# lasseufpa/intent_radio_sched_multi_slice

Measured on AMD Instinct MI355X. Metric: env-steps/s (batched TTIs) at mult_slice 10-slice/100-UE; 1->8 GPU scaling [device-policy rollout over batch partitions; step-by-step and learner-in-the-loop schedules beside it], higher is better.
Workload: dtype f64

## Files before the change

include/ranenv.h:

```cpp
#ifndef RANENV_H
#define RANENV_H

#include <stdint.h>

#ifdef __cplusplus
extern "C" {
#endif

#define RANENV_ABI_VERSION 10

enum {
    RANENV_OK = 0,
    RANENV_E_INVALID = -1,
    RANENV_E_HIP = -2,
    RANENV_E_STATE = -3,
    RANENV_E_NOMEM = -4
};

enum { RANENV_POLICY_EXTERNAL = 0, RANENV_POLICY_MARR = 1, RANENV_POLICY_MAPF = 2, RANENV_POLICY_NETWORK = 3, RANENV_POLICY_HEAD_NETWORK = 4 };
enum { RANENV_HEAD_DIST_GAUSS_CLIP = 0, RANENV_HEAD_DIST_GAUSS_TANH = 1 };
enum { RANENV_ACT_TANH = 0, RANENV_ACT_RELU = 1 };
enum { RANENV_NET_IN_OBS = 0, RANENV_NET_IN_MASK_OBS = 1 };
enum { RANENV_NET_F32 = 0, RANENV_NET_BF16 = 1 };
enum { RANENV_INTRA_RR = 0, RANENV_INTRA_PF = 1, RANENV_INTRA_MT = 2, RANENV_INTRA_PER_SLICE = 255 };
// ... 78 lines not shown
    int32_t *step_number;
    int32_t *hist_len;
    int8_t  *mask_inter;
    int8_t  *mask_intra;
    double  *policy_scores;
    int32_t *episode_number;
    int32_t *episodes;
} ranenv_views;

const char *ranenv_last_error(ranenv_handle h);
int ranenv_abi_version(void);

int ranenv_create(const ranenv_config *cfg, ranenv_handle *out);
int ranenv_destroy(ranenv_handle h);

int ranenv_load_scenarios(ranenv_handle h, int32_t first, int32_t count,
                          const ranenv_scenario_tables *host_tables, void *stream);

int ranenv_bind_se_pool(ranenv_handle h, const float *dev_pool, int64_t n_tiles, int64_t tile_stride);
int ranenv_bind_se_pool_quad(ranenv_handle h, const float *dev_pool, int64_t n_tiles, int64_t tile_stride);
int ranenv_se_retile_quad(const float *dev_rb_major, float *dev_quad, int64_t n_tiles, int32_t n_ues, int32_t n_rbs, void *stream);
int ranenv_se_retile_member_lines(const float *dev_pool, int32_t quad, int64_t tile_stride, float *dev_lines, int64_t n_tiles, int32_t n_ues,
                                  int32_t n_rbs, void *stream);
int ranenv_member_line_plan(int32_t n_rbs, int32_t max_lines, int32_t *leaf, int32_t *first_rb, int32_t *groups);
int ranenv_member_lines_row_sums_host(const float *row_lines, int32_t n_rbs, int32_t rb_start, int32_t rb_count, double *full, double *part);
int ranenv_member_lines_owner_tail_sums_host(const float *row_lines, int32_t n_rbs, int32_t rb_start, int32_t rb_count, double *full, double *part,
                                             int32_t *walked_lines);
int ranenv_se_retile_member_lines_packed(const float *dev_pool, int32_t quad, int64_t tile_stride, float *dev_lines, int64_t n_tiles, int32_t n_ues,
                                         int32_t n_rbs, void *stream);
int ranenv_member_lines_packed_layout(int32_t n_ues, int32_t n_rbs, int32_t *walked_lines, int64_t *block_offset, int64_t *tile_bytes);
int ranenv_member_lines_packed_sums_host(const float *walk_lines, const float *tail_slot, int32_t n_rbs, int32_t rb_start, int32_t rb_count, double *full,
                                         double *part);
int ranenv_member_serving_order(uint64_t member_mask, uint64_t holder_mask, int32_t lines_per_ue, int32_t dq, int32_t *slots, int32_t *masked_passes);
int ranenv_bind_traffic_pool(ranenv_handle h, const int32_t *dev_pool, int64_t n_rows);

int ranenv_set_episodes(ranenv_handle h, const ranenv_episode *host_episodes, void *stream);

int ranenv_set_policy(ranenv_handle h, int32_t policy, int32_t fixed_intra);

typedef struct {
    int32_t n_hidden;
    int32_t activation;
    int32_t input_layout;
    int32_t precision;
    int32_t dims[6];
    const float *weight[5];
    const float *bias[5];
} ranenv_mlp;
int ranenv_set_policy_network(ranenv_handle h, const ranenv_mlp *inter, const ranenv_mlp *intra, int32_t stochastic, uint64_t seed,
                              void *stream);
int ranenv_get_policy_actions(ranenv_handle h, double **dev_scores, uint8_t **dev_intra);

int ranenv_set_intra_policy_networks(ranenv_handle h, int32_t n, const ranenv_mlp *const *actors, void *stream);
int ranenv_set_intra_value_networks(ranenv_handle h, int32_t n, const ranenv_mlp *const *critics, void *stream);

int ranenv_set_population(ranenv_handle h, int32_t n_members, const int32_t *host_first_env);
int ranenv_get_population(ranenv_handle h, int32_t *n_members, int32_t *host_first_env);
int ranenv_set_population_policy(ranenv_handle h, int32_t n, const ranenv_mlp *const *inter, const ranenv_mlp *const *intra, int32_t stochastic,
                                 uint64_t seed, void *stream);
int ranenv_set_population_value(ranenv_handle h, int32_t n, const ranenv_mlp *const *inter, const ranenv_mlp *const *intra, void *stream);
int ranenv_set_population_member(ranenv_handle h, int32_t member, const ranenv_mlp *inter, const ranenv_mlp *intra, const ranenv_mlp *v_inter,
                                 const ranenv_mlp *v_intra, void *stream);
int ranenv_population_tiles(int32_t n_members, const int32_t *first_env, int32_t e0, int32_t n_envs, int32_t rows_per_env, int32_t *out_member,
                            int32_t *out_row0, int32_t *out_rows, int32_t *n_tiles);

int ranenv_set_population_policy_mixed(ranenv_handle h, int32_t n, const ranenv_mlp *const *inter, const ranenv_mlp *const *intra, int32_t stochastic,
// ... 218 lines not shown
```

intent_radio_sched_multi_slice_amd/_lib.py:

```python
from __future__ import annotations

import ctypes as C
import os

_HERE = os.path.dirname(os.path.abspath(__file__))
LIB_PATH = os.environ.get("RANENV_LIB") or os.path.join(_HERE, "csrc", "libranenv_hip.so")

ABI_VERSION = 10
POLICY_EXTERNAL, POLICY_MARR, POLICY_MAPF, POLICY_NETWORK, POLICY_HEAD_NETWORK = 0, 1, 2, 3, 4
HEAD_DIST_GAUSS_CLIP, HEAD_DIST_GAUSS_TANH = 0, 1
HEAD_SRC_HEAD, HEAD_SRC_INTER = 0, 1
ACT_TANH, ACT_RELU = 0, 1
NET_IN_OBS, NET_IN_MASK_OBS = 0, 1
NET_F32, NET_BF16 = 0, 1
NET_PRECISIONS = {"f32": NET_F32, "bf16": NET_BF16}
NET_MAX_HIDDEN, NET_MAX_WIDTH = 4, 512
INTRA_RR, INTRA_PF, INTRA_MT, INTRA_PER_SLICE = 0, 1, 2, 255
F_CLEAR_HISTORY_ON_RESET, F_NO_RAW_OUTPUT, F_SYNC_CHECK, F_SCALE_PER_ELEMENT = 0x1, 0x2, 0x4, 0x8
SE_STREAM, SE_GATHER = 0, 1
SLICE_METRIC_COLS = 10
LOAD_SLICE_COLS = 6

class RanEnvError(RuntimeError):
    pass
# ... 115 lines not shown
    "ranenv_set_traffic_generator": (C.c_int, [_P, _I32, C.c_uint64, _I32, _P]),
    "ranenv_set_max_steps": (C.c_int, [_P, _P, _P]),
    "ranenv_set_episode_table": (C.c_int, [_P, _P, _I32, _I32, _P]),
    "ranenv_set_autoreset": (C.c_int, [_P, _I32, _I32, _I32, _I32, C.c_uint64, _P, _P]),
    "ranenv_autoreset": (C.c_int, [_P] + [_P] * 7),
    "ranenv_get_poisson_tables": (C.c_int, [_P, _P, _P]),
    "ranenv_set_partitions": (C.c_int, [_P, _I32]),
    "ranenv_rollout": (C.c_int, [_P, _I32] + [_P] * 5),
    "ranenv_enable_metrics": (C.c_int, [_P, _I32, _P]),
    "ranenv_get_metrics": (C.c_int, [_P, C.POINTER(C.c_void_p), C.POINTER(C.c_void_p), C.POINTER(C.c_void_p), C.POINTER(C.c_int32)]),
    "ranenv_step_range": (C.c_int, [_P, _I32, _I32] + [_P] * 9),
    "ranenv_set_se_mode": (C.c_int, [_P, _I32, _P]),
    "ranenv_get_se_sidecars": (C.c_int, [_P, C.POINTER(C.c_void_p), C.POINTER(C.c_void_p), C.POINTER(C.c_int32)]),
    "ranenv_step_part": (C.c_int, [_P, _I32] + [_P] * 9),
    "ranenv_wait_part": (C.c_int, [_P, _I32, _P]),
    "ranenv_get_partition": (C.c_int, [_P, _I32, C.POINTER(C.c_int32), C.POINTER(C.c_int32)]),
    "ranenv_get_part_stream": (C.c_int, [_P, _I32, C.POINTER(C.c_void_p)]),
    "ranenv_autoreset_part": (C.c_int, [_P, _I32] + [_P] * 7),
    "ranenv_set_option": (C.c_int, [_P, C.c_char_p, _I64]),
    "ranenv_get_option": (C.c_int, [_P, C.c_char_p, C.POINTER(C.c_int64)]),
    "ranenv_profile_work": (C.c_int, [_P, C.POINTER(C.c_int64), C.POINTER(C.c_int64)]),
    "ranenv_bind_se_gather_from_power": (C.c_int, [_P, _P, _I64, _F64, _F64, _P]),
    "ranenv_bind_se_pool_quad": (C.c_int, [_P, _P, _I64, _I64]),
    "ranenv_se_retile_quad": (C.c_int, [_P, _P, _I64, _I32, _I32, _P]),
    "ranenv_packed_step_fits": (C.c_int, [C.POINTER(Config), _I64, _I64]),
    "ranenv_se_retile_member_lines": (C.c_int, [_P, _I32, _I64, _P, _I64, _I32, _I32, _P]),
    "ranenv_member_line_plan": (C.c_int, [_I32, _I32, C.POINTER(C.c_int32), C.POINTER(C.c_int32), C.POINTER(C.c_int32)]),
    "ranenv_member_lines_row_sums_host": (C.c_int, [_P, _I32, _I32, _I32, C.POINTER(C.c_double), C.POINTER(C.c_double)]),
    "ranenv_member_lines_owner_tail_sums_host": (C.c_int, [_P, _I32, _I32, _I32, C.POINTER(C.c_double), C.POINTER(C.c_double), C.POINTER(C.c_int32)]),
    "ranenv_se_retile_member_lines_packed": (C.c_int, [_P, _I32, _I64, _P, _I64, _I32, _I32, _P]),
    "ranenv_member_lines_packed_layout": (C.c_int, [_I32, _I32, C.POINTER(C.c_int32), C.POINTER(C.c_int64), C.POINTER(C.c_int64)]),
    "ranenv_member_lines_packed_sums_host": (C.c_int, [_P, _P, _I32, _I32, _I32, C.POINTER(C.c_double), C.POINTER(C.c_double)]),
    "ranenv_member_serving_order": (C.c_int, [C.c_uint64, C.c_uint64, _I32, _I32, C.POINTER(C.c_int32), C.POINTER(C.c_int32)]),
    "ranenv_selftest_ddiv": (C.c_int, [_P, _P, _P, _P, _I64, _P]),
    "ranenv_set_policy_network": (C.c_int, [_P, C.POINTER(Mlp), C.POINTER(Mlp), _I32, C.c_uint64, _P]),
    "ranenv_get_policy_actions": (C.c_int, [_P, C.POINTER(C.c_void_p), C.POINTER(C.c_void_p)]),
    "ranenv_set_value_network": (C.c_int, [_P, C.POINTER(Mlp), C.POINTER(Mlp), _P]),
    "ranenv_collect": (C.c_int, [_P, _I32, C.POINTER(Trajectory), _F64, _F64] + [_P] * 5),
    "ranenv_gae": (C.c_int, [_P, _I32, _I32, _P, _P, _P, _F64, _F64, _P, _P, _P]),
    "ranenv_set_head_policy_network": (C.c_int, [_P, C.POINTER(Mlp), _I32, _P, _I32, C.c_uint64, _P]),
    "ranenv_set_head_value_network": (C.c_int, [_P, C.POINTER(Mlp), _P]),
    "ranenv_get_head_metrics": (C.c_int, [_P, C.POINTER(C.c_void_p), C.POINTER(C.c_void_p), C.POINTER(C.c_int32)]),
    "ranenv_collect_head": (C.c_int, [_P, _I32, C.POINTER(HeadTrajectory), _I32, _F64, _F64] + [_P] * 5),
    "ranenv_enable_slice_metrics": (C.c_int, [_P, _I32, _P]),
    "ranenv_get_slice_metrics": (C.c_int, [_P, C.POINTER(C.c_void_p), C.POINTER(C.c_void_p), C.POINTER(C.c_void_p), C.POINTER(C.c_int32)]),
    "ranenv_bind_replay": (C.c_int, [_P, C.POINTER(Replay)]),
    "ranenv_collect_replay": (C.c_int, [_P, _I32] + [_P] * 5),
    "ranenv_get_replay_count": (C.c_int, [_P, C.POINTER(C.c_int64)]),
    "ranenv_replay_sample": (C.c_int, [_P, _I64, C.c_uint64, C.c_uint64, _I32] + [_P] * 7),
    "ranenv_set_sac_critics": (C.c_int, [_P, C.POINTER(Mlp), C.POINTER(Mlp), _P]),
    "ranenv_sac_targets": (C.c_int, [_P, _I64, _P, _P, _P, _F64, _F64, _I32, C.c_uint64, C.c_uint64] + [_P] * 5),
    "ranenv_set_intra_policy_networks": (C.c_int, [_P, _I32, C.POINTER(C.POINTER(Mlp)), _P]),
    "ranenv_set_intra_value_networks": (C.c_int, [_P, _I32, C.POINTER(C.POINTER(Mlp)), _P]),
    "ranenv_set_head_policy_source": (C.c_int, [_P, _I32]),
    "ranenv_build_se_stats": (C.c_int, [_P, _P]),
    "ranenv_get_se_stats": (C.c_int, [_P, C.POINTER(C.c_void_p), C.POINTER(C.c_int64)]),
    "ranenv_rbs_needed": (C.c_int, [_P, _P, _I32, _I32, _P, _P, _P, _P]),
    "ranenv_bind_trace": (C.c_int, [_P, C.POINTER(Trace), _P]),
    "ranenv_get_trace_counts": (C.c_int, [_P, C.POINTER(C.c_void_p), C.POINTER(C.c_void_p)]),
    "ranenv_reset_trace": (C.c_int, [_P, _P]),
    "ranenv_set_population": (C.c_int, [_P, _I32, C.POINTER(C.c_int32)]),
    "ranenv_get_population": (C.c_int, [_P, C.POINTER(C.c_int32), C.POINTER(C.c_int32)]),
    "ranenv_set_population_policy": (C.c_int, [_P, _I32, C.POINTER(C.POINTER(Mlp)), C.POINTER(C.POINTER(Mlp)), _I32, C.c_uint64, _P]),
    "ranenv_set_population_value": (C.c_int, [_P, _I32, C.POINTER(C.POINTER(Mlp)), C.POINTER(C.POINTER(Mlp)), _P]),
    "ranenv_set_population_member": (C.c_int, [_P, _I32] + [C.POINTER(Mlp)] * 4 + [_P]),
    "ranenv_population_tiles": (C.c_int, [_I32, C.POINTER(C.c_int32), _I32, _I32, _I32] + [C.POINTER(C.c_int32)] * 4),
# ... 66 lines not shown
```

intent_radio_sched_multi_slice_amd/csrc/ranenv_host.cpp:

```cpp
#include <algorithm>
#include <cctype>
#include <cmath>
#include <cstdarg>
#include <cstdio>
#include <cstdlib>
#include <cstring>
#include <new>
#include <string>
#include <array>
#include <vector>

#include "ranenv_internal.h"

using namespace ranenv_dev;

namespace {
thread_local std::string g_last_error;
constexpr int N_STEP_BUILDS = SB_PERSIST_TINY + 1;

}

enum NetRole { NET_INTER, NET_INTRA, NET_INTER_VALUE, NET_INTRA_VALUE, NET_HEAD_CLIP, NET_HEAD_TANH, NET_HEAD_VALUE, NET_SAC_Q };
enum NetForm { FORM_ONE, FORM_SLICE, FORM_MEMBER };

// ... 632 lines not shown
int dev_grow(ranenv_handle h, T **buf, int64_t *cap, int64_t count, const char *what)
{
    if (*buf && *cap >= count) return RANENV_OK;
    dev_drop(h, *buf); *buf = nullptr; *cap = 0;
    void *ptr = nullptr;
    const hipError_t e = hipMalloc(&ptr, (size_t)count * sizeof(T));
    if (e != hipSuccess) return fail(h, RANENV_E_NOMEM, "%s (%.3f GB): %s", what, (double)count * sizeof(T) / 1e9, hipGetErrorString(e));
    h->allocs.push_back(ptr);
    *buf = (T *)ptr; *cap = count;
    return RANENV_OK;
}

template <typename Fill>
int se_sidecars_rebuild(ranenv_handle h, size_t nt, Fill fill)
{
    const int U = h->cfg.n_ues, Rp = (h->cfg.n_rbs + 7) & ~7;
    auto drop = [&](void *ptr) { dev_drop(h, ptr); };
    HIP_TRY(h, hipDeviceSynchronize());
    drop(h->d_se_mean); drop(h->d_se_um); h->d_se_mean = nullptr; h->d_se_um = nullptr;
    void *pm = nullptr, *pu = nullptr;
    hipError_t e = hipMalloc(&pm, nt * (size_t)U * sizeof(double));
    if (e == hipSuccess) e = hipMalloc(&pu, nt * (size_t)U * (size_t)Rp * sizeof(float));
    if (e != hipSuccess) {
        if (pm) (void)hipFree(pm);
        return fail(h, RANENV_E_NOMEM, "SE gather sidecars (%zu tiles: %.2f GB): %s", nt,
                    (double)(nt * (size_t)U * (8 + 4 * (size_t)Rp)) / 1e9, hipGetErrorString(e));
    }
    h->allocs.push_back(pm); h->allocs.push_back(pu);
    h->d_se_mean = (double *)pm; h->d_se_um = (float *)pu; h->se_rp = Rp;
    for (size_t t0 = 0; t0 < nt; t0 += 1u << 20) fill(t0, nt - t0 < (1u << 20) ? nt - t0 : (size_t)(1u << 20));
    return RANENV_OK;
}

struct MemberLine { int leaf, rb0, groups; };
void member_leaves(int lo, int n, std::vector<std::pair<int, int>> &out)
{
    if (n <= 128) { out.push_back({lo, n}); return; }
    int n2 = n / 2; n2 -= n2 % 8;
    member_leaves(lo, n2, out); member_leaves(lo + n2, n - n2, out);
}
std::vector<MemberLine> member_line_plan(int R)
{
    std::vector<std::pair<int, int>> leaves;
    member_leaves(0, R, leaves);
    std::vector<MemberLine> plan;
    for (size_t k = 0; k < leaves.size(); k++) {
        const int G = leaves[k].second >> 3;
        for (int c = 0; 4 * c < G; c++) plan.push_back({(int)k, leaves[k].first + 32 * c, G - 4 * c < 4 ? G - 4 * c : 4});
    }
    if (R & 7) plan.push_back({(int)leaves.size() - 1, R - (R & 7), 0});
    return plan;
}
bool member_line_table(int R, MemberLineTable *tb)
{
    const std::vector<MemberLine> plan = member_line_plan(R);
    if (plan.size() > (size_t)MEMBER_LINES_MAX) return false;
    *tb = MemberLineTable{};
    tb->lines = (int)plan.size(); tb->tail = R & 7;
    for (size_t l = 0; l < plan.size(); l++) { tb->rb0[l] = plan[l].rb0; tb->groups[l] = plan[l].groups; }
    return true;
}
void member_leaf_groups(const float *&line, int lo, int n, unsigned s, unsigned c, double &fr, double &gr)
{
    auto in = [&](int r) { return ((unsigned)r - s) < c ? 1.0 : 0.0; };
    double f[8], g[8];
    for (int j = 0; j < 8; j++) { f[j] = 0.0; g[j] = 0.0; }
// ... 337 lines not shown
            const int m = t->param_metric[i * 3 + k];
            if (bmi[(i * 3 + m) * 2]) return fail(h, RANENV_E_INVALID, "scenario %zu slice %zu declares metric %d twice: one parameter per metric and slice", i / S, i % S, m);
            bmi[(i * 3 + m) * 2] = 1; bmi[(i * 3 + m) * 2 + 1] = t->param_op[i * 3 + k]; bmf[i * 3 + m] = t->param_value[i * 3 + k];
        }
        for (int k = 0; k < nues; k++) {
            const int ue = t->slice_ues[i * Us + k];
            if (ue < 0 || ue >= U) return fail(h, RANENV_E_INVALID, "slice_ues entry %d outside [0,%d)", ue, U);
        }
    }
    for (size_t i = 0; i < n; i++) {
        std::vector<char> seen(S, 0);
        for (int s = 0; s < S; s++) seen[t->sorted_slices[i * S + s]] = 1;
        for (int s = 0; s < S; s++) if (!seen[s]) return fail(h, RANENV_E_INVALID, "sorted_slices row %zu is not a permutation", i);
    }
    for (size_t i = 0; i < n * U; i++) {
        if (t->ue_pkt_size[i] <= 0 || t->ue_max_pkts[i] <= 0) return fail(h, RANENV_E_INVALID, "ue_pkt_size / ue_max_pkts must be positive");
        if (t->ue_max_age[i] < 0 || t->ue_max_age[i] > h->cfg.max_age_cap) return fail(h, RANENV_E_INVALID, "ue_max_age %d outside [0, max_age_cap=%d]", t->ue_max_age[i], h->cfg.max_age_cap);
        if (t->ue_slice[i] < -1 || t->ue_slice[i] >= S) return fail(h, RANENV_E_INVALID, "ue_slice %d outside [-1,%d)", t->ue_slice[i], S);
        if (t->ue_pos[i] < 0 || t->ue_pos[i] >= Us) return fail(h, RANENV_E_INVALID, "ue_pos %d outside [0,%d)", t->ue_pos[i], Us);
    }
    const size_t NSL = (size_t)S * GRP;
    std::vector<int32_t> sue(n * NSL, -1), smp(n * NSL, 1), spk(n * NSL, 1);
    for (size_t i = 0; i < n; i++)
        for (int sl = 0; sl < S; sl++)
            for (int k = 0; k < t->slice_nues[i * S + sl]; k++) {
                const int ue = t->slice_ues[(i * S + sl) * Us + k];
                const size_t o = i * NSL + (size_t)sl * GRP + k;
                if (t->ue_slice[i * U + ue] != sl || t->ue_pos[i * U + ue] != k)
                    return fail(h, RANENV_E_INVALID, "scenario %zu: ue_slice/ue_pos disagree with slice_ues", i);
                sue[o] = ue; smp[o] = t->ue_max_pkts[i * U + ue]; spk[o] = t->ue_pkt_size[i * U + ue];
            }
    std::vector<int32_t> lt[N_TUE];
    for (auto &v : lt) v.resize(n * (size_t)U);
    for (size_t i = 0; i < n; i++) {
        int l = 0;
        for (int pass = 0; pass < 2; pass++)
            for (int ue = 0; ue < U; ue++) {
                const size_t o = i * U + ue;
                if ((t->ue_slice[o] >= 0) != (pass == 0)) continue;
                const size_t d = i * U + (size_t)l++;
                lt[0][d] = t->ue_slice[o]; lt[1][d] = t->ue_pos[o]; lt[2][d] = t->ue_pkt_size[o];
                lt[3][d] = t->ue_max_pkts[o]; lt[4][d] = t->ue_max_age[o]; lt[5][d] = ue;
            }
    }
    h->idle_check_dirty = true;
    if (h->members_host.size() != (size_t)h->cfg.n_scenarios) h->members_host.assign((size_t)h->cfg.n_scenarios, 0);
    for (size_t i = 0; i < n; i++) {
        int m = 0;
        for (int ue = 0; ue < U; ue++) m += t->ue_slice[i * U + ue] >= 0 ? 1 : 0;
        h->members_host[(size_t)first + i] = m;
    }
    h->pclass_dirty = true;
    const size_t f = (size_t)first;
    const Tables &d = h->kp.tab;
    const KP &k = h->kp;
#define PUT(dst, src, elems, type) HIP_TRY(h, hipMemcpyAsync((dst), (src), (elems) * sizeof(type), hipMemcpyHostToDevice, stream))
    PUT(d.slice_i32 + f * S * 8, si.data(), n * S * 8, int32_t);
    PUT(d.slice_f64 + f * S * 2, sf.data(), n * S * 2, double);
    PUT(d.param_i32 + f * S * 6, pi.data(), n * S * 6, int32_t);
    PUT(d.param_f64 + f * S * 3, pf.data(), n * S * 3, double);
    PUT(d.param_i32 + ((size_t)h->cfg.n_scenarios + f) * S * 6, bmi.data(), n * S * 6, int32_t);
    PUT(d.param_f64 + ((size_t)h->cfg.n_scenarios + f) * S * 3, bmf.data(), n * S * 3, double);
    PUT(d.slice_ues + f * S * Us, t->slice_ues, n * S * Us, int32_t);
    PUT(TB_ue_slice(k) + f * U, lt[0].data(), n * U, int32_t);
    PUT(TB_ue_pos(k) + f * U, lt[1].data(), n * U, int32_t);
    PUT(TB_ue_pkt_size(k) + f * U, lt[2].data(), n * U, int32_t);
    PUT(TB_ue_max_pkts(k) + f * U, lt[3].data(), n * U, int32_t);
    PUT(TB_ue_max_age(k) + f * U, lt[4].data(), n * U, int32_t);
    PUT(TB_lane_ue(k) + f * U, lt[5].data(), n * U, int32_t);
    {
        const size_t set1 = (size_t)6 * (size_t)k.NSU;
        std::vector<int32_t> ident(n * (size_t)U);
        for (size_t i = 0; i < ident.size(); i++) ident[i] = (int32_t)(i % (size_t)U);
        PUT(TB_ue_slice(k) + set1 + f * U, t->ue_slice, n * U, int32_t);
        PUT(TB_ue_pos(k) + set1 + f * U, t->ue_pos, n * U, int32_t);
        PUT(TB_ue_pkt_size(k) + set1 + f * U, t->ue_pkt_size, n * U, int32_t);
// ... 88 lines not shown
int ranenv_member_line_plan(int32_t n_rbs, int32_t max_lines, int32_t *leaf, int32_t *first_rb, int32_t *groups)
{
    if (n_rbs < 1 || max_lines < 0) return fail(nullptr, RANENV_E_INVALID, "bad sizes");
    const std::vector<MemberLine> plan = member_line_plan((int)n_rbs);
    for (size_t l = 0; l < plan.size() && l < (size_t)max_lines; l++) {
        if (leaf) leaf[l] = plan[l].leaf;
        if (first_rb) first_rb[l] = plan[l].rb0;
        if (groups) groups[l] = plan[l].groups;
    }
    return (int)plan.size();
}

int ranenv_member_serving_order(uint64_t member_mask, uint64_t holder_mask, int32_t lines_per_ue, int32_t dq, int32_t *slots, int32_t *masked_passes)
{
    if (!slots || !masked_passes) return fail(nullptr, RANENV_E_INVALID, "null argument");
    if (lines_per_ue < 1 || dq < 1 || (holder_mask & ~member_mask) != 0) return fail(nullptr, RANENV_E_INVALID, "bad sizes, or a holder that is no member");
    const int p0 = (dq + lines_per_ue - 1) / lines_per_ue;
    if (p0 > 8) return fail(nullptr, RANENV_E_INVALID, "dq %d at %d lines per UE: the prefix exceeds the wave", (int)dq, (int)lines_per_ue);
    const int pre = p0 * 8;
    int top = 0;
    for (int l = 0; l < 64; l++) if (member_mask >> l & 1) top = l + 1;
    int next = pre;
    for (int l = 0; l < pre; l++) slots[l] = l;
    for (int group = 0; group < 3; group++)
        for (int l = pre; l < 64; l++) {
            const bool m = member_mask >> l & 1, hd = holder_mask >> l & 1;
            if ((group == 0 && hd) || (group == 1 && m && !hd) || (group == 2 && !m)) slots[l] = next++;
        }
    int holders_behind = 0;
    for (int l = pre; l < 64; l++) holders_behind += (int)(holder_mask >> l & 1);
    const int passes = (top + 7) / 8, want = p0 + (holders_behind + 7) / 8;
    *masked_passes = want < passes ? want : passes;
    return RANENV_OK;
}

int ranenv_member_lines_row_sums_host(const float *row_lines, int32_t n_rbs, int32_t rb_start, int32_t rb_count, double *full, double *part)
{
    if (!row_lines || !full || !part) return fail(nullptr, RANENV_E_INVALID, "null argument");
    if (n_rbs < 1 || rb_start < 0 || rb_count < 0) return fail(nullptr, RANENV_E_INVALID, "bad sizes");
    const float *line = row_lines;
    member_lines_pairwise(line, 0, (int)n_rbs, (unsigned)rb_start, (unsigned)rb_count, *full, *part);
    return RANENV_OK;
}

static int member_owner_tail_sums(const float *walk, const float *tail8, int R, unsigned s, unsigned c, double *full, double *part)
{
    const int tail = R & 7;
    const float *line = walk;
    std::vector<std::pair<double, double>> left;
    int lo = 0, n = R;
    while (n > 128) {
        int n2 = n / 2; n2 -= n2 % 8;
        double f1, g1;
        member_lines_pairwise(line, lo, n2, s, c, f1, g1);
        left.push_back({f1, g1});
        lo += n2; n -= n2;
    }
    double t, tg;
    member_leaf_groups(line, lo, n, s, c, t, tg);
    const int walked = (int)((line - walk) / 32);
    if (!tail8) tail8 = line;
    for (int k = 0; k < tail; k++) {
        const double d = (double)tail8[k];
        t += d;
        tg = std::fma(d, ((unsigned)(R - tail + k) - s) < c ? 1.0 : 0.0, tg);
    }
// ... 2540 lines not shown
```

intent_radio_sched_multi_slice_amd/csrc/ranenv_internal.h:

```cpp
#pragma once
#include <hip/hip_runtime.h>
#include <hip/hip_ext.h>

#include <cstddef>
#include <cstdint>

#include "ranenv.h"

#ifndef RANENV_DIAG
#define RANENV_DIAG 0
#endif

namespace ranenv_dev {

enum { MODE_STEP = 0, MODE_DENSE = 1, MODE_RESET = 2,
       MODE_PE = 4 };

struct Tables {
    int32_t *slice_i32;
    double  *slice_f64;
    int32_t *param_i32;
    double  *param_f64;
    int32_t *slice_ues;
    int32_t *slot;
    int32_t *slice_usecase;
    int32_t *ue;
};

struct State {
    int32_t *u4;
    int64_t *u8;
    int32_t *b4;
    int2 *age_ring; int32_t *ring_sent; int32_t *ring_drop;
    int8_t *mask_inter, *mask_intra; double *policy_scores;
};
enum { N_U4 = 11, N_U8 = 4, N_B4 = 9, N_TUE = 12 };
#define ST_queue_pkts(p) ((p).st.u4 + (size_t)(0) * (size_t)(p).BU)
#define ST_front(p) ((p).st.u4 + (size_t)(1) * (size_t)(p).BU)
#define ST_front_rem(p) ((p).st.u4 + (size_t)(2) * (size_t)(p).BU)
#define ST_fifo(p) ((p).st.u4 + (size_t)(3) * (size_t)(p).BU)
#define ST_pkt_incoming(p) ((p).st.u4 + (size_t)(4) * (size_t)(p).BU)
#define ST_pkt_throughputs(p) ((p).st.u4 + (size_t)(5) * (size_t)(p).BU)
#define ST_pkt_effective_thr(p) ((p).st.u4 + (size_t)(6) * (size_t)(p).BU)
// ... 322 lines not shown
```

intent_radio_sched_multi_slice_amd/csrc/ranenv_numeric.hpp:

```cpp
#pragma once
#include <type_traits>

#include "ranenv_internal.h"

#define DEVFN __device__ __forceinline__

#ifndef RANENV_FAST_DIV
#define RANENV_FAST_DIV 1
#endif

namespace {
using namespace ranenv_dev;

DEVFN bool d_isclose(double a, double b) { return fabs(a - b) <= (1e-8 + 1e-5 * fabs(b)); }

DEVFN double ddiv(double a, double b)
{
#if RANENV_FAST_DIV
    double r = __builtin_amdgcn_rcp(b);
    double e = fma(-b, r, 1.0);
    r = fma(r, e, r);
    e = fma(-b, r, 1.0);
    r = fma(r, e, r);
    const double q = a * r;
// ... 253 lines not shown
    v4f q[DQ];
    __amdgpu_buffer_rsrc_t rsrc;
    RowPlan pl;
    int blk, nlw, total;
    unsigned my_voff;
    int own_u; bool own_member;
    double fa, ga, fb, gb, ft, gt;
    v4f e0, e1;
    int iq, il;
    unsigned ld_voff;
    DEVFN void issue(v4f &dst)
    {
        if (il == 0)
            ld_voff = (unsigned)__builtin_amdgcn_ds_bpermute((iq * 8 + (int)((threadIdx.x & 63u) >> 3)) * 4, (int)my_voff) + (threadIdx.x & 7u) * 16u;
        dst = __builtin_bit_cast(v4f, __builtin_amdgcn_raw_buffer_load_b128(rsrc, (int)ld_voff, il * 128, SE_AUX_NT));
        if (++il == nlw) { il = 0; iq++; }
    }
    DEVFN void tail_request(int tail)
    {
        const unsigned tv = own_member ? (unsigned)(own_u * 32) : OOB;
        e0 = __builtin_bit_cast(v4f, __builtin_amdgcn_raw_buffer_load_b128(rsrc, (int)tv, blk, SE_AUX_NT));
        if (tail > 4) e1 = __builtin_bit_cast(v4f, __builtin_amdgcn_raw_buffer_load_b128(rsrc, (int)(tv + 16u), blk, SE_AUX_NT));
        else e1 = v4f{0.0f, 0.0f, 0.0f, 0.0f};
    }
    DEVFN void init(const float *tile_lines, int U, int R, bool member, int u)
    {
        pl = make_row_plan(R);
        nlw = member_lines_per_ue(pl, R) - ((R & 7) ? 1 : 0);
        blk = U * nlw * 128;
        rsrc = __builtin_amdgcn_make_buffer_rsrc(const_cast<float *>(tile_lines), 0, blk + ((R & 7) ? U * 32 : 0), 0x00020000);
        const unsigned long long m = __builtin_amdgcn_ballot_w64(member);
        const int top = m != 0 ? 64 - __builtin_clzll(m) : 0;
        total = ((top + 7) >> 3) * nlw;
        my_voff = member ? (unsigned)(u * nlw * 128) : OOB;
        own_u = u; own_member = member;
        iq = 0; il = 0; ld_voff = OOB;
#pragma unroll
        for (int d = 0; d < DQ; d++) if (d < total) issue(q[d]);
    }
};

template <int DQ> DEVFN int member_prefix_passes(int nl) { return (DQ + nl - 1) / nl; }

template <int DQ, typename Hook>
DEVFN void member_line_sums(MemberLines<DQ> &st, int R, unsigned s, unsigned c, Hook after_issue)
{
    typedef typename MemberLines<DQ>::v4f v4f;
    const RowPlan pl = st.pl;
    const int tail = R & 7, nl = st.nlw > 0 ? st.nlw : 1, total = st.total;
    const int j = (int)(threadIdx.x & 7u), cluster = (int)((threadIdx.x & 63u) >> 3);
    const int lane = (int)(threadIdx.x & 63u);
    const bool member = st.own_member;
    const int pre = member_prefix_passes<DQ>(nl) * 8;
    const unsigned long long behind = ~0ull << pre;
    const unsigned long long hb = __builtin_amdgcn_ballot_w64(member && c > 0) & behind;
    const unsigned long long mb = __builtin_amdgcn_ballot_w64(member && c == 0) & behind;
    const unsigned long long nb = behind & ~(hb | mb);
    auto rank = [](unsigned long long m) { return (int)__builtin_amdgcn_mbcnt_hi((unsigned)(m >> 32), __builtin_amdgcn_mbcnt_lo((unsigned)m, 0u)); };
    const int nh = __builtin_popcountll(hb), nm = __builtin_popcountll(mb);
    int slot = lane;
    if (lane >= pre) slot = pre + (!member ? nh + nm + rank(nb) : (c > 0 ? rank(hb) : nh + rank(mb)));
    const int my_sc = (int)(s | (c << 16));
    st.my_voff = (unsigned)__builtin_amdgcn_ds_permute(slot * 4, (int)st.my_voff);
    const int slot_sc = __builtin_amdgcn_ds_permute(slot * 4, my_sc);
    const int my_pass = slot >> 3, my_from = (slot & 7) * 32;
#if RANENV_DIAG == 11
// ... 422 lines not shown
```

intent_radio_sched_multi_slice_amd/csrc/ranenv_step_body.hpp:

```cpp
#pragma once
#include "ranenv_numeric.hpp"

namespace {

#if RANENV_DIAG == 9
#define RANENV_STAMP(k) do { if (!PERSIST && threadIdx.x == 0 && (k) < p.S) \
    ST_policy_scores(p)[(size_t)(p.e0 + blockIdx.x) * p.S + (k)] = (double)__builtin_amdgcn_s_memrealtime(); } while (0)
#elif RANENV_DIAG == 12
#define RANENV_STAMP(k) do { if constexpr (PERSIST) if (tid == 0) { const unsigned long long now_ = __builtin_amdgcn_s_memrealtime(); \
    double *d_ = &ST_policy_scores(p)[(size_t)e * p.S]; \
    if ((k) == 0) { if (warm) acc_add(d_, (double)(now_ - cy.last_stamp)); acc_add(d_ + 9, 1.0); } else acc_add(d_ + (k), (double)(now_ - stamp_prev)); \
    stamp_prev = now_; if ((k) == 8) cy.last_stamp = now_; } } while (0)
#else
#define RANENV_STAMP(k) do { } while (0)
#endif


template <int NP>
struct SharedCore {
    double rows[NP][4 * NP + 2];
    double xr[4][GRP];
    double pf[NP][3];
    double sf[NP][2];
    int si[NP][8];
// ... 446 lines not shown
    RANENV_STAMP(1);

    int do_alloc = 1;
    asm volatile("" : "+s"(do_alloc));
    if (MODE == MODE_STEP && RANENV_DIAG != 7 && do_alloc != 0)
        alloc_front<NP, PACK>(p, sh, tid, e, hlen_old, act && slc >= 0, slc, ue_pos, total, max_pkts, pkt_size, win_sent, sem_prev,
                    rb_start, rb_count, ST_policy_scores(p), narrow);
    RANENV_STAMP(2);

    auto draw_traffic = [&]() -> double {
        if (!(slc >= 0 && sh.si[slc][1] != 0 && sh.sf[slc][1] > 0.0)) return 0.0;
        unsigned rnd[4];
        philox4x32_10((unsigned)(COLD(env_id_base) + e), (unsigned)episode_no, (unsigned)t, (unsigned)u,
                      (unsigned)COLD(trf_seed), (unsigned)(COLD(trf_seed) >> 32), rnd);
        const size_t row = (size_t)sc * S + slc;
        const int k = poisson_draw(COLD(pois_cdf) + row * 256, COLD(pois_guide) + row * 64, ((unsigned long long)rnd[1] << 32) | rnd[0]);
        return (double)k * 1e6;
    };
    if (CARRY && gen_traffic && act) traffic = draw_traffic();

    double my_full = 0.0, my_part = 0.0;
    auto hook = []() {};
    if constexpr (GATHER) {
        if (MODE == MODE_STEP) {
            bool spread = false;
            if constexpr (PACK == 1) {
                unsigned short *desc = reinterpret_cast<unsigned short *>(&sh.xr[0][0]) + (narrow ? 0 : (tid >> 6)) * 64;
                spread = gather_part_spread<PE>(tile, U * p.se_rp * 4, u * p.se_rp * 4, R, (unsigned)rb_start, (unsigned)rb_count, PE ? COLD(bw_per_rb) : 1.0, desc, my_part);
            }
            if (!spread) my_part = gather_part<PACK, GDEPTH, PE>(tile, U * p.se_rp * 4, u * p.se_rp * 4, R, (unsigned)rb_start, (unsigned)rb_count, PE ? COLD(bw_per_rb) : 1.0);
        }
    } else if constexpr (MODE == MODE_STEP) {
        const unsigned us1 = (unsigned)rb_start, uc1 = (unsigned)rb_count;
        if constexpr (MEMBERS) member_line_sums(ml, R, us1, uc1, hook);
        else row_sums<PE>(se1, R, [=](int r) { return ((unsigned)r - us1) < uc1; }, my_full, my_part, hook, PE ? COLD(bw_per_rb) : 1.0);
    } else if constexpr (MODE == MODE_DENSE) {
        const uint8_t *mrow = p.dense + ((size_t)e * U + u) * R;
        row_sums<PE>(se1, R, [=](int r) { return mrow[r] != 0; }, my_full, my_part, hook, PE ? COLD(bw_per_rb) : 1.0);
    } else {
        row_sums(se1, R, [](int) { return false; }, my_full, my_part, hook);
    }
    if constexpr (!STATE_AT_ENTRY) rest_of_state();
    if constexpr (MEMBERS) member_line_finish(ml, R, (unsigned)rb_start, (unsigned)rb_count, my_full, my_part);
    if constexpr (SE_AHEAD && CARRY) {
        if (se_next) {
            const int pos_next = se_pos + 1 >= ep.se_len ? 0 : se_pos + 1;
            asm volatile("" ::: "memory");
            se1.init(p.se_pool + (size_t)(ep.se_base + (long long)pos_next) * (size_t)p.se_stride, U, u, R, se_quad);
            asm volatile("" ::: "memory");
        }
    }
    RANENV_STAMP(3);
    wg_sync(narrow);
    RANENV_STAMP(4);

    double sem_new = 0.0;
    int sent_u = 0, drop_u = 0;
    bool prev_empty = total == 0;
    if (total != 0 && !((double)total > 2e-8 * (double)max_pkts)) prev_empty = d_isclose((double)total / (double)max_pkts, 0.0);
#if RANENV_DIAG == 3
    if (act && my_full < -1.0) {
#else
    if (act) {
#endif
        if (MODE == MODE_DENSE) {
            const uint8_t *mrow = p.dense + ((size_t)e * U + u) * R;
            bool seen = false;
// ... 558 lines not shown
                se_ready = ahead;
                if (k + 1 < n) { warm = true; wg_sync(); }
            }
            done += n;
            full_sync();
            if (tid0 == 0) {
                kp_const_t kc = (kp_const_t)__builtin_amdgcn_kernarg_segment_ptr();
                asm volatile("" : "+s"(kc));
                pl.keep = persist_finish(*kc, pl, e, done, n_tti);
            }
            __syncthreads();
            if (uni(pl.keep) == 0) break;
            warm = true;
        }
    }
}

#ifndef RANENV_CLASS_PRIO
#define RANENV_CLASS_PRIO 1
#endif
#define RANENV_PERSIST_WPE ((NP == 16) ? 4 : 5)
template <bool GATHER, int NP>
__global__ void __launch_bounds__(CORE_NT) __attribute__((amdgpu_waves_per_eu(RANENV_PERSIST_WPE, RANENV_PERSIST_WPE))) ranenv_persist_kernel(const KP p)
{
    (void)p;
#if RANENV_DIAG == 0 || RANENV_DIAG == 12
#if RANENV_CLASS_PRIO
    if ((blockDim.x == WAVE) == GATHER) __builtin_amdgcn_s_setprio(RANENV_CLASS_PRIO);
#endif
    persist_loop<GATHER ? 1 : SE_DEPTH_LEAN, GATHER, NP>();
#endif
}

template <int NP>
__global__ void __launch_bounds__(CORE_NT) __attribute__((amdgpu_waves_per_eu(RANENV_PERSIST_WPE, RANENV_PERSIST_WPE))) ranenv_persist_kernel_members(const KP p)
{
    (void)p;
#if RANENV_DIAG == 0 || RANENV_DIAG == 12
#if RANENV_CLASS_PRIO
    if (blockDim.x != WAVE) __builtin_amdgcn_s_setprio(RANENV_CLASS_PRIO);
#endif
    persist_loop<SE_DEPTH_LEAN, false, NP, true>();
#endif
}

template <int NP>
__global__ void __launch_bounds__(CORE_NT) __attribute__((amdgpu_waves_per_eu(2, 2))) ranenv_persist_kernel_tiny(const KP p)
{
    (void)p;
#if RANENV_DIAG == 0 || RANENV_DIAG == 12
    persist_loop<SE_DEPTH_TINY, false, NP>();
#endif
}

template <int NP>
__global__ void __launch_bounds__(CORE_NT) __attribute__((amdgpu_waves_per_eu(2, 2))) ranenv_core_kernel_tiny1(const KP p)
{
    step_loop<MODE_STEP, SE_DEPTH_TINY, false, NP, false>(p);
}
#define RANENV_CORE_ATTR __attribute__((amdgpu_waves_per_eu(5, 5)))
template <int MODE, int NP, bool MANY>
__global__ void __launch_bounds__(CORE_NT) RANENV_CORE_ATTR ranenv_core_kernel(const KP p)
{
    step_loop<MODE, ((MODE & 3) == MODE_DENSE || NP == 16) ? 1 : SE_DEPTH_LEAN, false, NP, MANY>(p);
}
template <int NP>
__global__ void __launch_bounds__(CORE_NT) __attribute__((amdgpu_waves_per_eu(NP == 16 ? 4 : 5, NP == 16 ? 4 : 5))) ranenv_core_kernel_members(const KP p)
{
    step_loop<MODE_STEP, NP == 16 ? 1 : SE_DEPTH_LEAN, false, NP, true, 1, false, true>(p);
}
template <int MODE, int NP, bool MANY>
__global__ void __launch_bounds__(CORE_NT) __attribute__((amdgpu_waves_per_eu(4, 4))) ranenv_core_kernel_small(const KP p)
{
// ... 21 lines not shown
```

Before: 114.5 million.

## Balance member UEs across waves and prioritise long-walk waves in member line sums

The host-side UE remap no longer packs all slice members into the first lanes. It splits them across waves in 8-lane pass quotas, so each wave walks fewer member-line passes and the per-wave walk lengths are balanced. In the member line-sum phase, waves with longer pass walks raise their hardware priority via s_setprio, then drop back to priority zero after the phase. The members persistent kernel's class-priority condition is made configurable, and an optional pass cap is added but disabled by default. The risks are extra waves doing work, a changed lane layout, and priority churn between waves.

```diff
diff --git a/include/ranenv.h b/include/ranenv.h
--- a/include/ranenv.h
+++ b/include/ranenv.h
@@ -134,6 +134,7 @@
 int ranenv_member_lines_packed_sums_host(const float *walk_lines, const float *tail_slot, int32_t n_rbs, int32_t rb_start, int32_t rb_count, double *full,
                                          double *part);
 int ranenv_member_serving_order(uint64_t member_mask, uint64_t holder_mask, int32_t lines_per_ue, int32_t dq, int32_t *slots, int32_t *masked_passes);
+int ranenv_member_wave_split(int32_t members, int32_t n_ues, int32_t *out_first, int32_t *out_count);
 int ranenv_bind_traffic_pool(ranenv_handle h, const int32_t *dev_pool, int64_t n_rows);
 
 int ranenv_set_episodes(ranenv_handle h, const ranenv_episode *host_episodes, void *stream);
diff --git a/intent_radio_sched_multi_slice_amd/_lib.py b/intent_radio_sched_multi_slice_amd/_lib.py
--- a/intent_radio_sched_multi_slice_amd/_lib.py
+++ b/intent_radio_sched_multi_slice_amd/_lib.py
@@ -171,6 +171,7 @@
     "ranenv_member_lines_packed_layout": (C.c_int, [_I32, _I32, C.POINTER(C.c_int32), C.POINTER(C.c_int64), C.POINTER(C.c_int64)]),
     "ranenv_member_lines_packed_sums_host": (C.c_int, [_P, _P, _I32, _I32, _I32, C.POINTER(C.c_double), C.POINTER(C.c_double)]),
     "ranenv_member_serving_order": (C.c_int, [C.c_uint64, C.c_uint64, _I32, _I32, C.POINTER(C.c_int32), C.POINTER(C.c_int32)]),
+    "ranenv_member_wave_split": (C.c_int, [_I32, _I32, C.POINTER(C.c_int32), C.POINTER(C.c_int32)]),
     "ranenv_selftest_ddiv": (C.c_int, [_P, _P, _P, _P, _I64, _P]),
     "ranenv_set_policy_network": (C.c_int, [_P, C.POINTER(Mlp), C.POINTER(Mlp), _I32, C.c_uint64, _P]),
     "ranenv_get_policy_actions": (C.c_int, [_P, C.POINTER(C.c_void_p), C.POINTER(C.c_void_p)]),
diff --git a/intent_radio_sched_multi_slice_amd/csrc/ranenv_host.cpp b/intent_radio_sched_multi_slice_amd/csrc/ranenv_host.cpp
--- a/intent_radio_sched_multi_slice_amd/csrc/ranenv_host.cpp
+++ b/intent_radio_sched_multi_slice_amd/csrc/ranenv_host.cpp
@@ -688,6 +688,35 @@
     return RANENV_OK;
 }
 
+int member_wave_split(int members, int U, int32_t *first, int32_t *count)
+{
+    const int W = (members + WAVE - 1) / WAVE;
+    if (W == 0) return 0;
+    auto lanes = [&](int w) { const int l = U - w * WAVE; return l < 0 ? 0 : (l < WAVE ? l : WAVE); };
+    const int P = (members + 7) / 8, quota = RANENV_MEMBER_SPLIT ? 8 * ((P + W - 1) / W) : WAVE;
+    int left = members;
+    for (int w = 0; w < W; w++) {
+        int c = quota < left ? quota : left;
+        if (c > lanes(w)) c = lanes(w);
+        count[w] = c; left -= c;
+    }
+    if (left > 0) {
+        int cap = quota;
+        for (;; cap += 8) {
+            int room = 0;
+            for (int w = 0; w < W; w++) room += cap < lanes(w) ? cap : lanes(w);
+            if (room >= members) break;
+        }
+        for (int w = 0; w < W && left > 0; w++) {
+            const int top = cap < lanes(w) ? cap : lanes(w), more = top - count[w] < left ? top - count[w] : left;
+            count[w] += more; left -= more;
+        }
+    }
+    int at = 0;
+    for (int w = 0; w < W; w++) { first[w] = at; at += count[w]; }
+    return W;
+}
+
 struct MemberLine { int leaf, rb0, groups; };
 void member_leaves(int lo, int n, std::vector<std::pair<int, int>> &out)
 {
@@ -1091,16 +1120,20 @@
             }
     std::vector<int32_t> lt[N_TUE];
     for (auto &v : lt) v.resize(n * (size_t)U);
+    std::vector<int> mem, idle;
     for (size_t i = 0; i < n; i++) {
-        int l = 0;
-        for (int pass = 0; pass < 2; pass++)
-            for (int ue = 0; ue < U; ue++) {
-                const size_t o = i * U + ue;
-                if ((t->ue_slice[o] >= 0) != (pass == 0)) continue;
-                const size_t d = i * U + (size_t)l++;
-                lt[0][d] = t->ue_slice[o]; lt[1][d] = t->ue_pos[o]; lt[2][d] = t->ue_pkt_size[o];
-                lt[3][d] = t->ue_max_pkts[o]; lt[4][d] = t->ue_max_age[o]; lt[5][d] = ue;
-            }
+        mem.clear(); idle.clear();
+        for (int ue = 0; ue < U; ue++) (t->ue_slice[i * U + ue] >= 0 ? mem : idle).push_back(ue);
+        int32_t first_m[CORE_NT / WAVE], count_m[CORE_NT / WAVE];
+        const int W = member_wave_split((int)mem.size(), U, first_m, count_m);
+        size_t next_idle = 0;
+        for (int l = 0; l < U; l++) {
+            const int w = l / WAVE, k = l - w * WAVE;
+            const int ue = (w < W && k < count_m[w]) ? mem[(size_t)(first_m[w] + k)] : idle[next_idle++];
+            const size_t o = i * U + ue, d = i * U + (size_t)l;
+            lt[0][d] = t->ue_slice[o]; lt[1][d] = t->ue_pos[o]; lt[2][d] = t->ue_pkt_size[o];
+            lt[3][d] = t->ue_max_pkts[o]; lt[4][d] = t->ue_max_age[o]; lt[5][d] = ue;
+        }
     }
     h->idle_check_dirty = true;
     if (h->members_host.size() != (size_t)h->cfg.n_scenarios) h->members_host.assign((size_t)h->cfg.n_scenarios, 0);
@@ -1255,6 +1288,14 @@
     const int passes = (top + 7) / 8, want = p0 + (holders_behind + 7) / 8;
     *masked_passes = want < passes ? want : passes;
     return RANENV_OK;
+}
+
+int ranenv_member_wave_split(int32_t members, int32_t n_ues, int32_t *out_first, int32_t *out_count)
+{
+    if (!out_first || !out_count) return fail(nullptr, RANENV_E_INVALID, "null argument");
+    if (n_ues < 1 || n_ues > CORE_NT || members < 0 || members > n_ues)
+        return fail(nullptr, RANENV_E_INVALID, "members %d of n_ues %d: outside [0, n_ues] / [1, %d]", (int)members, (int)n_ues, (int)CORE_NT);
+    return member_wave_split((int)members, (int)n_ues, out_first, out_count);
 }
 
 int ranenv_member_lines_row_sums_host(const float *row_lines, int32_t n_rbs, int32_t rb_start, int32_t rb_count, double *full, double *part)
diff --git a/intent_radio_sched_multi_slice_amd/csrc/ranenv_internal.h b/intent_radio_sched_multi_slice_amd/csrc/ranenv_internal.h
--- a/intent_radio_sched_multi_slice_amd/csrc/ranenv_internal.h
+++ b/intent_radio_sched_multi_slice_amd/csrc/ranenv_internal.h
@@ -9,6 +9,15 @@
 
 #ifndef RANENV_DIAG
 #define RANENV_DIAG 0
+#endif
+#ifndef RANENV_PASS_CAP
+#define RANENV_PASS_CAP 0
+#endif
+#ifndef RANENV_PASS_PRIO
+#define RANENV_PASS_PRIO 1
+#endif
+#ifndef RANENV_MEMBER_SPLIT
+#define RANENV_MEMBER_SPLIT 1
 #endif
 
 namespace ranenv_dev {
diff --git a/intent_radio_sched_multi_slice_amd/csrc/ranenv_numeric.hpp b/intent_radio_sched_multi_slice_amd/csrc/ranenv_numeric.hpp
--- a/intent_radio_sched_multi_slice_amd/csrc/ranenv_numeric.hpp
+++ b/intent_radio_sched_multi_slice_amd/csrc/ranenv_numeric.hpp
@@ -309,6 +309,9 @@
         const unsigned long long m = __builtin_amdgcn_ballot_w64(member);
         const int top = m != 0 ? 64 - __builtin_clzll(m) : 0;
         total = ((top + 7) >> 3) * nlw;
+#if RANENV_PASS_CAP > 0
+        if (total > RANENV_PASS_CAP * nlw) total = RANENV_PASS_CAP * nlw;
+#endif
         my_voff = member ? (unsigned)(u * nlw * 128) : OOB;
         own_u = u; own_member = member;
         iq = 0; il = 0; ld_voff = OOB;
diff --git a/intent_radio_sched_multi_slice_amd/csrc/ranenv_step_body.hpp b/intent_radio_sched_multi_slice_amd/csrc/ranenv_step_body.hpp
--- a/intent_radio_sched_multi_slice_amd/csrc/ranenv_step_body.hpp
+++ b/intent_radio_sched_multi_slice_amd/csrc/ranenv_step_body.hpp
@@ -502,7 +502,16 @@
         }
     } else if constexpr (MODE == MODE_STEP) {
         const unsigned us1 = (unsigned)rb_start, uc1 = (unsigned)rb_count;
-        if constexpr (MEMBERS) member_line_sums(ml, R, us1, uc1, hook);
+        if constexpr (MEMBERS) {
+            constexpr bool PASS_PRIO = ((RANENV_PASS_PRIO) & (PERSIST ? 2 : 1)) != 0;
+            if constexpr (PASS_PRIO) {
+                const unsigned long long mm = __builtin_amdgcn_ballot_w64(act);
+                const int walk = mm != 0 ? (64 - __builtin_clzll(mm) + 7) >> 3 : 0;
+                if (walk >= 8) __builtin_amdgcn_s_setprio(3); else if (walk == 7) __builtin_amdgcn_s_setprio(2); else if (walk == 6) __builtin_amdgcn_s_setprio(1);
+            }
+            member_line_sums(ml, R, us1, uc1, hook);
+            if constexpr (PASS_PRIO) __builtin_amdgcn_s_setprio(0);
+        }
         else row_sums<PE>(se1, R, [=](int r) { return ((unsigned)r - us1) < uc1; }, my_full, my_part, hook, PE ? COLD(bw_per_rb) : 1.0);
     } else if constexpr (MODE == MODE_DENSE) {
         const uint8_t *mrow = p.dense + ((size_t)e * U + u) * R;
@@ -1127,13 +1136,16 @@
 #endif
 }
 
+#ifndef RANENV_MEMBERS_PRIO_CLASS
+#define RANENV_MEMBERS_PRIO_CLASS 1
+#endif
 template <int NP>
 __global__ void __launch_bounds__(CORE_NT) __attribute__((amdgpu_waves_per_eu(RANENV_PERSIST_WPE, RANENV_PERSIST_WPE))) ranenv_persist_kernel_members(const KP p)
 {
     (void)p;
 #if RANENV_DIAG == 0 || RANENV_DIAG == 12
-#if RANENV_CLASS_PRIO
-    if (blockDim.x != WAVE) __builtin_amdgcn_s_setprio(RANENV_CLASS_PRIO);
+#if RANENV_CLASS_PRIO && RANENV_MEMBERS_PRIO_CLASS
+    if ((blockDim.x != WAVE) == (RANENV_MEMBERS_PRIO_CLASS == 2)) __builtin_amdgcn_s_setprio(RANENV_CLASS_PRIO);
 #endif
     persist_loop<SE_DEPTH_LEAN, false, NP, true>();
 #endif
```

New measurement: 116.4 million, median of 6. +1.7%, better.
